# AtharvRN/dflash

Measured on AMD Instinct MI355X. Metric: accepted_tokens_per_sec, higher is better.
Workload: dtype bf16

## Files before the change

### dflash_amd/_lib.py

```python
from __future__ import annotations

import ctypes as C
import os

import torch

HERE = os.path.dirname(os.path.abspath(__file__))
LIB_PATH = os.environ.get("DFL_LIB_PATH") or os.path.join(HERE, "lib", "libdflash_hip.so")

_p, _i, _i64, _f, _u64 = C.c_void_p, C.c_int, C.c_int64, C.c_float, C.c_uint64


class Rows(C.Structure):
    _fields_ = [("frag", C.c_void_p), ("rows", C.c_void_p), ("ld", C.c_int64), ("ss", C.c_void_p),
                ("nss", C.c_int32), ("norm_w", C.c_void_p), ("eps", C.c_float), ("valid_word", C.c_int32),
                ("mode", C.c_int32)]


_r = C.POINTER(Rows)


class RowsBatch(C.Structure):
    _fields_ = [("r0", Rows), ("frag_stride", C.c_int64), ("rows_stride", C.c_int64), ("ss_stride", C.c_int64)]


_rb = C.POINTER(RowsBatch)

W_BF16, W_E4M3, W_BF16X13 = 0, 1, 2


class Weight(C.Structure):
    _fields_ = [("wp", C.c_void_p), ("scale", C.c_void_p), ("format", C.c_int32)]


_w = C.POINTER(Weight)

SIGNATURES = {
    "dfl_version": (_i, []),
    "dfl_last_error": (C.c_char_p, []),
    "dfl_pack_weight": (_i, [_p, _p, _i, _i, _p]),
    "dfl_pack_weight_gateup": (_i, [_p, _p, _p, _i, _i, _p]),
    "dfl_set_dyn": (_i, [_p, _i, _i, _i, _i, _p]),
    "dfl_set_dyn2": (_i, [_p, _i, _i, _i, _i, _p]),
# ... 114 lines not shown
```

### dflash_amd/csrc/gemm_skinny.hip

```cpp
#include "gemm_rows.h"
#include "dfl_rng.h"

namespace {

struct GemmArgs {
  const bf16x8 *wp;
  int KS;
  int ntiles;
  int nfr;
  int nch;
  int nhalf;
  int gx;
  const int32_t *dyn;
  RowSrc src[2];
  float *out;
  int ldo;
  bf16_t *act;
  const int32_t *elist, *n_active;
  int npp;
  int row0, nrows;
  int nrows_word;
  float *best_val;
  int *best_idx;
  float *best2_val;
// ... 49 lines not shown
  a.gx = (int)b.gx;
  a.nch = CHUNKED ? (int)b.nch_nss : 1;
  a.nrows_word = (int)b.nrows_word1 - 1;
  RowSrc &s = a.src[0];
  s.frag = reinterpret_cast<const bf16x8 *>(x);
  s.rows = reinterpret_cast<const bf16_t *>(x);
  s.ld = ld;
  s.ss = ss;
  s.nw = nw;
  s.mode = (int)b.mode;
  s.valid_word = (int)b.valid_word1 - 1;
  if (NORM) s.nss = (int)b.nch_nss;
  return a;
}

template <bool CHUNKED>
bool gemm_head(GemmHead &h, const GemmArgs &a) {
  const RowSrc &s = a.src[0];
  HeadBits b{};
  b.KS = a.KS;
  b.nfr = a.nfr;
  b.mode = s.mode;
  b.valid_word1 = s.valid_word < 0 ? 0 : s.valid_word + 1;
  b.nrows_word1 = a.nrows_word < 0 ? 0 : a.nrows_word + 1;
  b.gx = a.gx;
  b.nhalf = a.nhalf;
  const int nch_nss = CHUNKED ? a.nch : (s.mode == 2 ? s.nss : 0);
  b.nch_nss = nch_nss;
  const int64_t ld = s.mode == 0 ? 0 : s.ld;
  const bool fits = (int)b.KS == a.KS && (int)b.nfr == a.nfr && (int)b.mode == s.mode && (int)b.gx == a.gx &&
// ... 19 lines not shown
#ifdef DFL_GEMM_STAMPS
__device__ unsigned long long g_gstamps[8];
__device__ unsigned long long g_wgstamps[256][4];
#define GSTAMP(i)                                                                         \
  do {                                                                                    \
    if (threadIdx.x == 0 && blockIdx.x == 0 && blockIdx.y == 0) g_gstamps[i] = __builtin_amdgcn_s_memrealtime(); \
    if (threadIdx.x == 0 && blockIdx.y == 0 && blockIdx.x < 256 && ((i) == 0 || (i) == 4 || (i) == 5))            \
      g_wgstamps[blockIdx.x][(i) == 0 ? 0 : (i) - 3] = __builtin_amdgcn_s_memrealtime();                           \
  } while (0)
#else
#define GSTAMP(i)
#endif

constexpr int gemm_fr(int MT, bool CHUNKED) { return CHUNKED ? 4 : (MT == 1 ? 8 : 4); }

template <int MT, bool CHUNKED, int EPI, bool NORM, bool W8 = false, bool W13 = false>
__device__ __forceinline__ void gemm_body(const GemmArgs &a, const SampleArgs &sa) {
  GSTAMP(0);
  static_assert(!W13 || (MT == 1 && !W8), "W13: the single-tile bf16 kernels only");
  static_assert(!W13 || !CHUNKED || (EPI == EPI_RESID && !NORM), "W13, K-chunked: the residual launch only");
  constexpr int FR = gemm_fr(MT, CHUNKED);
  constexpr int NW = W13 ? (CHUNKED ? 3 : 6) : (W8 ? FR / 2 : FR);
  __shared__ float red[2][16][MT][256];
  __shared__ float ssred[NORM ? MT : 1][16][16];
  __shared__ bf16x8 nwl[NORM ? MT : 1][NORM ? 512 : 1];

  const int tid = threadIdx.x;
  const int w = __builtin_amdgcn_readfirstlane(tid >> 6);
  const int l = tid & 63;

  auto ks0_of = [&](int c) { return ((blockIdx.y * a.nch + c) * 16 + w) * a.nfr; };
  auto nf_of = [&](int c) {
    int nf = a.KS - ks0_of(c);
    return nf < 0 ? 0 : (nf > a.nfr ? a.nfr : nf);
  };

  const int stride = a.gx;
  constexpr bool SILU = EPI == EPI_SILU || EPI == EPI_SILU_E;
  constexpr bool moe = EPI == EPI_SILU_E;
  const int nwhole = (!SILU && (int)blockIdx.x < a.ntiles) ? (a.ntiles - 1 - (int)blockIdx.x) / stride + 1 : 0;
  const bool has_half = !SILU && (int)blockIdx.x < a.nhalf;
  const int myhalf = (int)blockIdx.x & 1;
  auto half_of = [&](int j) -> int { return (!SILU && j >= nwhole) ? myhalf : -1; };
  auto tile_of = [&](int j) -> int {
    if (!SILU) return j < nwhole ? (int)blockIdx.x + j * stride : a.ntiles + ((int)blockIdx.x >> 1);
    int p = (int)blockIdx.x + (j >> 1) * stride;
    if (moe) p = a.elist[p / a.npp] * a.npp + p % a.npp;
    return 2 * p + (j & 1);
  };

  bf16x8 wA[NW], wB[NW];
  float scA = 1.f, scB = 1.f;
  W13Extra exA{}, exB{};
  bf16x8 xA[MT][FR], xB[MT][FR];
  bf16x8 xr[MT][FR];

  const int nf0 = nf_of(0);
  const int ngroups = SILU ? a.ntiles >> 1 : a.ntiles;
  int nseq;
  if (SILU) {
    const int npairs = moe ? a.n_active[0] * a.npp : a.ntiles >> 1;
    nseq = (int)blockIdx.x < npairs ? 2 * ((npairs - 1 - (int)blockIdx.x) / stride + 1) : 0;
  } else {
    nseq = nwhole + (has_half ? 1 : 0);
  }
  const int nitems = nseq * a.nch;

  int nv[MT];
  auto read_nv = [&]() {
#pragma unroll
    for (int mt = 0; mt < MT; ++mt) {
      const RowSrc &s0 = a.src[mt];
      nv[mt] = (s0.valid_word >= 0 && a.dyn) ? a.dyn[s0.valid_word] : 16;
    }
  };

  float best = -INFINITY;
  int bestn = 0x7fffffff;
  float second = -INFINITY;
  float gate_sum = 0.f;
  int arg_rows = 0;
  int pos_row0 = 0, rng_extra = 0;

  auto load_item_x = [&](bf16x8(&xb)[MT][FR], int c) {
    const int ks0 = ks0_of(c);
    int ks[FR];
#pragma unroll
    for (int f = 0; f < FR; ++f) ks[f] = ks0 + f < a.KS ? ks0 + f : a.KS - 1;
    bf16x8 wv[MT][FR];
#pragma unroll
    for (int mt = 0; mt < MT; ++mt)
#pragma unroll
      for (int f = 0; f < FR; ++f) wv[mt][f] = xb[mt][f] = (bf16x8){0, 0, 0, 0, 0, 0, 0, 0};
#pragma unroll
    for (int mt = 0; mt < MT; ++mt) issue_x<FR, false>(a.src[mt], ks, l, nv[mt], xb[mt], wv[mt]);
  };
// ... 103 lines not shown
          const bool keep = ks0c + f < a.KS && (a.src[mt].mode == 0 || (l & 15) < nv[mt]);
          xv = keep ? xb[mt][f] : (bf16x8){0, 0, 0, 0, 0, 0, 0, 0};
        }
        bf16x8 wf;
        if constexpr (W13 && CHUNKED)
          wf = w13_frag(wr, ex.sg[0], ex.meta, f, l);
        else if constexpr (W13)
          wf = w13_frag(wr, ex, f, l);
        else
          wf = weight_frag<W8>(wr, f);
        acc[mt] = __builtin_amdgcn_mfma_f32_16x16x32_bf16(wf, xv, acc[mt], 0, 0, 0);
      }
    if (!CHUNKED || c == a.nch - 1) finish(t, pos, wsc);
  };

  const int first_tile = (SILU || nwhole > 0) ? (int)blockIdx.x : a.ntiles + ((int)blockIdx.x >> 1);
  const int first_half = (SILU || nwhole > 0) ? -1 : myhalf;
  const bool first_live = SILU ? (int)blockIdx.x < ngroups : (nwhole > 0 || has_half);
  auto ask_resid0 = [&]() {
    if (PREF) {
      const int ff = tid & 255;
      resid0 = a.h_io[(int64_t)(ff >> 4) * a.ldh + first_tile * 16 + (ff & 15)];
    }
  };

  read_nv();
  int arg_word = 0;
  const bool arg_dyn = (EPI == EPI_ARGMAX || EPI == EPI_SAMPLE) && a.dyn && a.nrows_word >= 0;
  if (arg_dyn) arg_word = a.dyn[a.nrows_word];
  if (EPI == EPI_SAMPLE) {
    const int base = sa.pos_dyn ? sa.pos_dyn[sa.pos_word] : sa.pos_base;
    pos_row0 = base + sa.pos_add;
    rng_extra = sa.rng_stream == (int)DFL_RNG_DRAFT ? base : 0;
// ... 87 lines not shown
        }
    }
    GSTAMP(2);
#pragma unroll
    for (int mt = 0; mt < MT; ++mt) {
      if (NORM)
        finish_xl<FR>(a.src[mt], ks, take, l, nv[mt], rstd[mt], raw[mt], nwl[mt], xr[mt]);
      else
        finish_x<FR, false>(a.src[mt], take, l, nv[mt], 1.f, raw[mt], wv0[mt], xr[mt]);
    }
  } else {
    if constexpr (W8)
      load_w8(wA, scA, first_tile, ks0_of(0), first_live ? nf0 : 0, first_half);
    else if constexpr (W13)
      load_w13(wA, exA, first_tile, ks0_of(0), first_live ? nf0 : 0, first_half, 0);
    else if (nitems > 0 || !moe)
      load_ksteps<FR>(wA, a.wp + ((size_t)first_tile * a.KS + ks0_of(0)) * 64, first_live ? nf0 : 0, l, first_half);
    GSTAMP(6);
    load_item_x(xA, 0);
    ask_resid0();
    GSTAMP(1);
    GSTAMP(2);
  }

  if (EPI == EPI_ARGMAX || EPI == EPI_SAMPLE) arg_rows = arg_dyn ? arg_word - a.row0 : a.nrows;
  GSTAMP(3);
  if (nitems > 0) {
    int j = 0, c = 0;
    for (int i = 0;; i += 2) {
      int jn = j, cn = c + 1;
      if (cn == a.nch) {
        cn = 0;
        ++jn;
      }
      if (i + 1 < nitems) load_item(wB, scB, exB, xB, tile_of(jn), cn, half_of(jn));
      process(wA, scA, exA, xA, tile_of(j), c, j);
      if (i == 0) GSTAMP(4);
      if (i + 1 >= nitems) break;
      int j2 = jn, c2 = cn + 1;
// ... 40 lines not shown
template <bool CHUNKED, int EPI, bool NORM>
__global__ __launch_bounds__(1024) void k_gemm_w8(GEMM_HEAD_PARAMS, GemmArgs rest) {
  gemm_body<1, CHUNKED, EPI, NORM, true>(with_head<CHUNKED, NORM>(rest, GEMM_HEAD_NAMES), SampleArgs{});
}

template <int EPI, bool NORM>
__global__ __launch_bounds__(1024) void k_gemm_w13(GEMM_HEAD_PARAMS, GemmArgs rest) {
  gemm_body<1, false, EPI, NORM, false, true>(with_head<false, NORM>(rest, GEMM_HEAD_NAMES), SampleArgs{});
}

template <int EPI>
__global__ __launch_bounds__(1024) void k_gemm_w13c(GEMM_HEAD_PARAMS, GemmArgs rest) {
  gemm_body<1, true, EPI, false, false, true>(with_head<true, false>(rest, GEMM_HEAD_NAMES), SampleArgs{});
}

template <bool NORM>
__global__ __launch_bounds__(1024) void k_gemm_s(GEMM_HEAD_PARAMS, GemmArgs rest, SampleArgs sa) {
  gemm_body<1, false, EPI_SAMPLE, NORM>(with_head<false, NORM>(rest, GEMM_HEAD_NAMES), sa);
}

template <bool NORM>
__global__ __launch_bounds__(1024) void k_gemm_s_w8(GEMM_HEAD_PARAMS, GemmArgs rest, SampleArgs sa) {
  gemm_body<1, false, EPI_SAMPLE, NORM, true>(with_head<false, NORM>(rest, GEMM_HEAD_NAMES), sa);
}

template <int MT, bool CHUNKED, int EPI, bool W8 = false>
bool launch_gemm(GemmArgs &a, dim3 grid, hipStream_t stream) {
  bool norm = false;
  for (int mt = 0; mt < MT; ++mt) norm |= a.src[mt].mode == 2;
  a.gx = (int)grid.x;
  GemmHead h;
  if (!gemm_head<CHUNKED>(h, a)) return false;
  if constexpr (W8) {
    static_assert(MT == 1, "the W8 kernels take one 16-row tile");
    if (!a.wscale || a.KS % 2 || a.nfr % 2) {
      dfl_set_error("skinny GEMM (fp8): needs a scale vector, K %% 64 == 0 and an even share per wave (K=%d, nfr=%d)",
                    a.KS * 32, a.nfr);
      return false;
    }
    if constexpr (!CHUNKED) {
      if (norm) {
        hipLaunchKernelGGL((k_gemm_w8<false, EPI, true>), grid, dim3(1024), 0, stream, GEMM_HEAD_OF(h), a);
        return true;
      }
    }
    hipLaunchKernelGGL((k_gemm_w8<CHUNKED, EPI, false>), grid, dim3(1024), 0, stream, GEMM_HEAD_OF(h), a);
    return true;
  }
  if constexpr (!CHUNKED) {
    if (norm) {
      hipLaunchKernelGGL((k_gemm<MT, false, EPI, true>), grid, dim3(1024), 0, stream, GEMM_HEAD_OF(h), a);
      return true;
    }
  }
  hipLaunchKernelGGL((k_gemm<MT, CHUNKED, EPI, false>), grid, dim3(1024), 0, stream, GEMM_HEAD_OF(h), a);
  return true;
}

static int64_t w13_quads_bytes(int N, int K) { return (int64_t)(N / 16) * (K / 128) * W13_QUAD_BYTES; }

template <int EPI>
bool launch_gemm_w13(const char *who, GemmArgs &a, const dfl_weight *w, int N, dim3 grid, hipStream_t stream) {
  if (w->scale) {
    dfl_set_error("%s: a DFL_W_BF16X13 weight takes no scale vector (the bases and patch words follow the codes)", who);
    return false;
  }
  if (a.KS % 64 || a.nfr % 4 || a.nfr * 16 != a.KS) {
    dfl_set_error("%s: DFL_W_BF16X13 covers K = 2048 and K = 4096 only (whole quads of four k-steps per wave; K=%d, %d k-steps "
                  "per wave)", who, a.KS * 32, a.nfr);
    return false;
  }
  a.wscale = reinterpret_cast<const float *>(reinterpret_cast<const char *>(w->wp) + w13_quads_bytes(N, a.KS * 32));
  a.gx = (int)grid.x;
  GemmHead h;
  if (!gemm_head<false>(h, a)) return false;
  if (a.src[0].mode == 2)
    hipLaunchKernelGGL((k_gemm_w13<EPI, true>), grid, dim3(1024), 0, stream, GEMM_HEAD_OF(h), a);
  else
    hipLaunchKernelGGL((k_gemm_w13<EPI, false>), grid, dim3(1024), 0, stream, GEMM_HEAD_OF(h), a);
  return true;
}

__global__ __launch_bounds__(64) void k_argmax_finish(const float *best_val, const int *best_idx, const float *best2_val,
                                                      int nblk, int row0, int nrows, const int32_t *dyn, int nrows_word,
                                                      int64_t *out_ids, int out_off, float *margin_out) {
  int rows = nrows;
  if (dyn && nrows_word >= 0) rows = dyn[nrows_word] - row0;
  const int m = row0 + blockIdx.x;
  if ((int)blockIdx.x >= rows) return;
  float bv = -INFINITY, sv = -INFINITY;
// ... 179 lines not shown
  a.out = out;
  a.ldo = N;
  int gx1 = 0;
  if (ksplit == 1) plan_tiles(a, N / 16, true, gx1);
  dim3 grid(ksplit == 1 ? gx1 : grid_x_for(a.ntiles, ksplit), ksplit);
  const bool ok = mt == 1 ? launch_gemm<1, false, EPI_F32>(a, grid, (hipStream_t)stream)
                          : launch_gemm<2, false, EPI_F32>(a, grid, (hipStream_t)stream);
  if (!ok) return DFL_EINVAL;
  DFL_CHECK_LAUNCH("dfl_gemm_f32");
  return DFL_OK;
}

namespace {
template <bool W8, bool W13 = false>
int gemm_silu_mul_impl(const char *who, const dfl_weight *w, const dfl_rows *x, int I, int K, void *act_frag,
                       const int32_t *dyn, void *stream) {
  DFL_REQUIRE(w->wp && act_frag && (!W8 || w->scale), "%s: null pointer", who);
  DFL_REQUIRE(I > 0 && K > 0 && I % 16 == 0 && K % (W8 ? 64 : 32) == 0, "%s: need I%%16==0, K%%%d==0", who, W8 ? 64 : 32);
  const int KS = K / 32;
  DFL_REQUIRE(KS <= 16 * 8, "%s: K=%d needs a K split, which the fused activation cannot take", who, K);
  GemmArgs a{};
  if (!fill_src(a.src[0], x, K, who)) return DFL_EINVAL;
  a.wp = (const bf16x8 *)w->wp;
  a.wscale = w->scale;
  a.dyn = dyn;
  a.KS = KS;
  a.ntiles = 2 * (I / 16);
  a.nfr = (KS + 15) / 16;
  if (W8) a.nfr += a.nfr & 1;
  a.nch = 1;
  a.act = (bf16_t *)act_frag;
  if constexpr (W13) {
    if (!launch_gemm_w13<EPI_SILU>(who, a, w, 2 * I, dim3(grid_x_for(I / 16), 1), (hipStream_t)stream)) return DFL_EINVAL;
  } else if (!launch_gemm<1, false, EPI_SILU, W8>(a, dim3(grid_x_for(I / 16), 1), (hipStream_t)stream)) {
    return DFL_EINVAL;
  }
  DFL_CHECK_LAUNCH(who);
  return DFL_OK;
}
}

extern "C" int dfl_gemm_silu_mul(const dfl_weight *w_gateup, const dfl_rows *x, int I, int K, void *act_frag,
                                 const int32_t *dyn, void *stream) {
  const char *who = "dfl_gemm_silu_mul";
  if (w_gateup && w_gateup->format == DFL_W_BF16X13)
    return gemm_silu_mul_impl<false, true>(who, w_gateup, x, I, K, act_frag, dyn, stream);
  if (!weight_ok(who, w_gateup)) return DFL_EINVAL;
  return w_gateup->format == DFL_W_BF16 ? gemm_silu_mul_impl<false>(who, w_gateup, x, I, K, act_frag, dyn, stream)
                                        : gemm_silu_mul_impl<true>(who, w_gateup, x, I, K, act_frag, dyn, stream);
}

extern "C" int dfl_gemm_silu_mul_experts(const void *wp_gateup, int64_t wp_expert_stride, const dfl_rows *x, int E, int I, int K,
                                         void *act_frag, int64_t act_expert_stride, const int32_t *list,
                                         const int32_t *n_active, const int32_t *dyn, void *stream) {
  DFL_REQUIRE(wp_gateup && act_frag && list && n_active, "dfl_gemm_silu_mul_experts: null pointer");
  DFL_REQUIRE(E >= 1 && E <= 1024 && I > 0 && K > 0 && I % 16 == 0 && K % 32 == 0, "dfl_gemm_silu_mul_experts: bad shape");
  DFL_REQUIRE(wp_expert_stride == (int64_t)2 * I * K && act_expert_stride == (int64_t)16 * I,
              "dfl_gemm_silu_mul_experts: the experts' weights and outputs must lie back to back (strides %lld, %lld)",
              (long long)wp_expert_stride, (long long)act_expert_stride);
  const int KS = K / 32;
  DFL_REQUIRE(KS <= 16 * 8, "dfl_gemm_silu_mul_experts: K=%d exceeds 4096", K);
  GemmArgs a{};
  if (!fill_src(a.src[0], x, K, "dfl_gemm_silu_mul_experts")) return DFL_EINVAL;
  a.wp = (const bf16x8 *)wp_gateup;
// ... 4 lines not shown
  a.nch = 1;
  a.act = (bf16_t *)act_frag;
  a.elist = list;
  a.n_active = n_active;
  a.npp = I / 16;
  if (!launch_gemm<1, false, EPI_SILU_E>(a, dim3(256, 1), (hipStream_t)stream)) return DFL_EINVAL;
  DFL_CHECK_LAUNCH("dfl_gemm_silu_mul_experts");
  return DFL_OK;
}

extern "C" int64_t dfl_argmax_ws_bytes(void) { return 256 * 16 * (int64_t)(2 * sizeof(float) + sizeof(int)); }

namespace {
int gemm_argmax_impl(const char *who, const dfl_weight *w, const dfl_rows *x, int V, int K, int row0, int nrows,
                     const int32_t *dyn, int nrows_dyn_word, void *ws, int64_t *out_ids, int out_off, void *logits,
                     float *margin_out, hipEvent_t ev0, hipEvent_t ev1, void *stream, const SampleArgs *smp = nullptr) {
  const bool w8 = w->format == DFL_W_E4M3, w13 = w->format == DFL_W_BF16X13;
  DFL_REQUIRE(w->wp && ws && out_ids && (!w8 || w->scale), "%s: null pointer", who);
  DFL_REQUIRE(V > 0 && K > 0 && V % 16 == 0 && K % (w8 ? 64 : 32) == 0, "%s: need V%%16==0, K%%%d==0 (V=%d K=%d)", who,
              w8 ? 64 : 32, V, K);
  DFL_REQUIRE(row0 >= 0 && nrows >= 0 && row0 + nrows <= 16, "%s: rows [%d,%d) outside the 16-row tile", who, row0,
              row0 + nrows);
  const int KS = K / 32;
  DFL_REQUIRE(KS <= 16 * 8, "%s: K=%d exceeds 4096 (argmax needs finished sums)", who, K);
  GemmArgs a{};
  if (!fill_src(a.src[0], x, K, who)) return DFL_EINVAL;
  a.wp = (const bf16x8 *)w->wp;
  a.dyn = dyn;
  a.KS = KS;
  a.ntiles = V / 16;
  a.nfr = (KS + 15) / 16;
// ... 13 lines not shown
  if (ev0) (void)hipEventRecord(ev0, (hipStream_t)stream);
  if (smp) {
    a.gx = gx;
    GemmHead h;
    if (!gemm_head<false>(h, a)) return DFL_EINVAL;
    if (w8) {
      if (a.src[0].mode == 2)
        hipLaunchKernelGGL(k_gemm_s_w8<true>, dim3(gx, 1), dim3(1024), 0, (hipStream_t)stream, GEMM_HEAD_OF(h), a, *smp);
      else
        hipLaunchKernelGGL(k_gemm_s_w8<false>, dim3(gx, 1), dim3(1024), 0, (hipStream_t)stream, GEMM_HEAD_OF(h), a, *smp);
    } else if (a.src[0].mode == 2)
      hipLaunchKernelGGL(k_gemm_s<true>, dim3(gx, 1), dim3(1024), 0, (hipStream_t)stream, GEMM_HEAD_OF(h), a, *smp);
    else
      hipLaunchKernelGGL(k_gemm_s<false>, dim3(gx, 1), dim3(1024), 0, (hipStream_t)stream, GEMM_HEAD_OF(h), a, *smp);
  } else if (w13) {
    if (!launch_gemm_w13<EPI_ARGMAX>(who, a, w, V, dim3(gx, 1), (hipStream_t)stream)) return DFL_EINVAL;
  } else if (w8) {
    if (!launch_gemm<1, false, EPI_ARGMAX, true>(a, dim3(gx, 1), (hipStream_t)stream)) return DFL_EINVAL;
  } else {
    if (!launch_gemm<1, false, EPI_ARGMAX>(a, dim3(gx, 1), (hipStream_t)stream)) return DFL_EINVAL;
  }
  if (ev1) (void)hipEventRecord(ev1, (hipStream_t)stream);
  hipLaunchKernelGGL(k_argmax_finish, dim3(16), dim3(64), 0, (hipStream_t)stream, a.best_val, a.best_idx, a.best2_val, gx,
                     row0, nrows, dyn, nrows_dyn_word, out_ids, out_off, margin_out);
  DFL_CHECK_LAUNCH(who);
  return DFL_OK;
}
}

extern "C" int dfl_gemm_argmax(const dfl_weight *w, const dfl_rows *x, int V, int K, int row0, int nrows,
                               const int32_t *dyn, int nrows_dyn_word, void *ws, int64_t *out_ids, int out_off,
                               void *logits, float *margin_out, void *ev_start, void *ev_end, void *stream) {
  const char *who = "dfl_gemm_argmax";
  if (!(w && w->format == DFL_W_BF16X13) && !weight_ok(who, w)) return DFL_EINVAL;
  return gemm_argmax_impl(who, w, x, V, K, row0, nrows, dyn, nrows_dyn_word, ws, out_ids, out_off, logits, margin_out,
                          (hipEvent_t)ev_start, (hipEvent_t)ev_end, stream);
}

extern "C" int dfl_gemm_sample(const dfl_weight *w, const dfl_rows *x, int V, int K, int row0, int nrows,
                               const int32_t *dyn, int nrows_dyn_word, void *ws, int64_t *out_ids, int out_off,
                               void *logits, float *margin_out, uint64_t seed, float inv_t, int rng_stream,
                               const int32_t *pos_dyn, int pos_word, int pos_base, int pos_add, void *stream) {
  const char *who = "dfl_gemm_sample";
  if (!weight_ok(who, w)) return DFL_EINVAL;
  DFL_REQUIRE(w->wp && (w->format == DFL_W_BF16 || w->scale) && ws && out_ids, "%s: null pointer", who);
  DFL_REQUIRE(inv_t > 0.f && inv_t <= 1e5f, "%s: inv_t=%g outside (0, 1e5]", who, (double)inv_t);
  DFL_REQUIRE(rng_stream == (int)DFL_RNG_TARGET || rng_stream == (int)DFL_RNG_DRAFT, "%s: unknown stream %d", who,
              rng_stream);
  DFL_REQUIRE(!pos_dyn || (pos_word >= 0 && pos_word < DFL_DYN_WORDS), "%s: pos_word=%d outside the record", who, pos_word);
  const SampleArgs smp{seed, inv_t, rng_stream, pos_dyn, pos_word, pos_base, pos_add};
  return gemm_argmax_impl(who, w, x, V, K, row0, nrows, dyn, nrows_dyn_word, ws, out_ids, out_off, logits, margin_out,
                          nullptr, nullptr, stream, &smp);
}


namespace {
template <bool W8, bool W13 = false>
int gemm_resid_impl(const char *who, const dfl_weight *w, const dfl_rows *x, int N, int K, void *h_io, int64_t ldh,
                    int add_residual, void *tap, int64_t ldtap, float *ss_out, const int32_t *dyn, void *stream) {
  DFL_REQUIRE(w->wp && h_io && (!W8 || w->scale), "%s: null pointer", who);
  DFL_REQUIRE(N > 0 && K > 0 && N % 16 == 0 && K % (W8 ? 64 : 32) == 0, "%s: need N%%16==0, K%%%d==0 (N=%d K=%d)", who,
              W8 ? 64 : 32, N, K);
  DFL_REQUIRE(ldh >= N && (!tap || ldtap >= N), "%s: row strides shorter than N", who);
  const int KS = K / 32;
  GemmArgs a{};
  if (!fill_src(a.src[0], x, K, who)) return DFL_EINVAL;
  a.wp = (const bf16x8 *)w->wp;
  a.wscale = w->scale;
  a.dyn = dyn;
  a.KS = KS;
  a.ntiles = N / 16;
  a.h_io = (bf16_t *)h_io;
  a.ldh = ldh;
  a.add_resid = add_residual ? 1 : 0;
  a.tap = (bf16_t *)tap;
  a.ldtap = ldtap;
  a.ss_out = ss_out;
  int gx = 0;
  plan_tiles(a, N / 16, KS <= 16 * 8 && !ss_out, gx);
  const dim3 grid(gx, 1);
  if (KS <= 16 * 8) {
    a.nfr = (KS + 15) / 16;
    if (W8) a.nfr += a.nfr & 1;
    a.nch = 1;
    if (!launch_gemm<1, false, EPI_RESID, W8>(a, grid, (hipStream_t)stream)) return DFL_EINVAL;
  } else {
    DFL_REQUIRE(a.src[0].mode != 2, "%s: a normalised source needs K <= 4096", who);
    a.nfr = 4;
    a.nch = (KS + 63) / 64;
    if constexpr (W13) {
      a.wscale = reinterpret_cast<const float *>(reinterpret_cast<const char *>(w->wp) + w13_quads_bytes(N, K));
      a.gx = (int)grid.x;
      GemmHead h;
      if (!gemm_head<true>(h, a)) return DFL_EINVAL;
      hipLaunchKernelGGL((k_gemm_w13c<EPI_RESID>), grid, dim3(1024), 0, (hipStream_t)stream, GEMM_HEAD_OF(h), a);
    } else if (!launch_gemm<1, true, EPI_RESID, W8>(a, grid, (hipStream_t)stream)) {
      return DFL_EINVAL;
    }
  }
  DFL_CHECK_LAUNCH(who);
  return DFL_OK;
}
}

extern "C" int dfl_gemm_resid(const dfl_weight *w, const dfl_rows *x, int N, int K, void *h_io, int64_t ldh,
                              int add_residual, void *tap, int64_t ldtap, float *ss_out, const int32_t *dyn,
                              void *stream) {
  const char *who = "dfl_gemm_resid";
  if (w && w->format == DFL_W_BF16X13 && K > 4096 && K % 2048 == 0) {
    DFL_REQUIRE(!w->scale, "%s: a DFL_W_BF16X13 weight takes no scale vector (the bases and patch words follow the codes)", who);
    return gemm_resid_impl<false, true>(who, w, x, N, K, h_io, ldh, add_residual, tap, ldtap, ss_out, dyn, stream);
  }
  if (!weight_ok(who, w)) return DFL_EINVAL;
  return w->format == DFL_W_BF16
             ? gemm_resid_impl<false>(who, w, x, N, K, h_io, ldh, add_residual, tap, ldtap, ss_out, dyn, stream)
             : gemm_resid_impl<true>(who, w, x, N, K, h_io, ldh, add_residual, tap, ldtap, ss_out, dyn, stream);
}
```

### dflash_amd/ops.py

```python
from __future__ import annotations

from types import SimpleNamespace
from typing import NamedTuple, Optional

import torch

from ._lib import W_BF16, W_BF16X13, W_E4M3, Rows, Weight, check, lib

BF16, F32, I32, I64 = torch.bfloat16, torch.float32, torch.int32, torch.int64
DYN_S, DYN_TAU, DYN_BS, DYN_POS0, DYN_START, DYN_STOP, DYN_CYCLE = range(7)


def _stream() -> int:
    return torch.cuda.current_stream().cuda_stream


def _p(t: Optional[torch.Tensor], dtype=None, name="tensor") -> Optional[int]:
    if t is None:
        return None
    if not t.is_cuda:
        raise RuntimeError(f"dflash_amd: {name} must be a GPU tensor (got {t.device}); there is no CPU path")
    if dtype is not None and t.dtype != dtype:
        raise TypeError(f"dflash_amd: {name} must be {dtype}, got {t.dtype}")
    if not t.is_contiguous():
# ... 225 lines not shown
    return hit[3]


def bf16x13_report() -> dict:
    live = [v for v in _x13_twins.values() if v[0]() is not None]
    return {"packed": sum(v[3] is not None for v in live), "kept_bf16": sum(v[3] is None for v in live),
            "patched_items": sum(v[4]["patched"] for v in live), "refused_items": sum(v[4]["refused"] for v in live)}


def check_stream_format(stream_format: str) -> bool:
    if stream_format not in STREAM_FORMATS:
        raise ValueError(f"stream_format must be one of {STREAM_FORMATS}, got {stream_format!r}")
    return stream_format == "auto"


def _w(wp, N: int, K: int, name: str) -> Weight:
    if isinstance(wp, Bf16x13Weight):
        if (wp.N, wp.K) != (N, K):
            raise ValueError(f"dflash_amd: {name} is a bf16x13 weight of {wp.N} x {wp.K}, the launch asks for {N} x {K}")
        return Weight(_p(wp.data, U8, name), None, W_BF16X13)
    if not isinstance(wp, Fp8Weight):
        return Weight(_p(wp, BF16, name), None, W_BF16)
    if (wp.N, wp.K) != (N, K):
        raise ValueError(f"dflash_amd: {name} is an fp8 weight of {wp.N} x {wp.K}, the launch asks for {N} x {K}")
    return Weight(_p(wp.wp, U8, name), _p(wp.scale, F32, name + ".scale"), W_E4M3)


def _we(wp, E: int, N: int, K: int, name: str):
    if not isinstance(wp, Fp8Experts):
        assert wp.dim() == 2 and wp.is_contiguous()
        return Weight(_p(wp, BF16, name), None, W_BF16), wp
    if (wp.E, wp.N, wp.K) != (E, N, K):
        raise ValueError(f"dflash_amd: {name} holds fp8 experts of {wp.E} x {wp.N} x {wp.K}, the launch asks for "
                         f"{E} x {N} x {K}")
    return Weight(_p(wp.wp, U8, name), _p(wp.scale, F32, name + ".scale"), W_E4M3), wp.wp


def set_dyn(dyn: torch.Tensor, S: int, tau: int, bs: int, pos0: int) -> None:
    check(lib().dfl_set_dyn(_p(dyn, I32, "dyn"), S, tau, bs, pos0, _stream()), "dfl_set_dyn")

# ... 73 lines not shown
    ntiles, ks_steps = N // 16, K // 32
    best, best_score = None, None
    for ks in range(min_ksplit(K, mt), 17):
        nfr = -(-ks_steps // (16 * ks))
        if nfr < 2 and ks > min_ksplit(K, mt):
            break
        gx_max = max(1, 256 // ks)
        per_wg = -(-ntiles // gx_max)
        fill = (ntiles * ks) / (256.0 * per_wg)
        score = (round(min(fill, 1.0), 3), min(per_wg, 2), -ks)
        if best_score is None or score > best_score:
            best, best_score = ks, score
    return best


def gemm_silu_mul(wp_gu, x, I: int, K: int, act_frag: torch.Tensor, dyn=None) -> None:
    assert act_frag.numel() >= 16 * I
    check(lib().dfl_gemm_silu_mul(_w(wp_gu, 2 * I, K, "wp_gu"), _src(x).ref, I, K, _p(act_frag, BF16, "act"),
                                  _p(dyn, I32, "dyn"), _stream()), "dfl_gemm_silu_mul")


def argmax_ws(device) -> torch.Tensor:
    return torch.empty(lib().dfl_argmax_ws_bytes(), dtype=torch.uint8, device=device)


def gemm_argmax(wp, x, V: int, K: int, row0: int, nrows: int, ws, out_ids: torch.Tensor, out_off: int = 0,
                dyn=None, nrows_dyn_word: int = -1, logits: Optional[torch.Tensor] = None,
                margins: Optional[torch.Tensor] = None, events=None) -> None:
    if logits is not None:
        assert logits.numel() >= 16 * V
    if margins is not None:
        assert margins.numel() >= out_off + nrows
    ev_start, ev_end = (None, None) if events is None else (events[0].cuda_event, events[1].cuda_event)
    check(lib().dfl_gemm_argmax(_w(wp, V, K, "wp"), _src(x).ref, V, K, row0, nrows, _p(dyn, I32, "dyn"), nrows_dyn_word,
                                _p(ws), _p(out_ids, I64, "out_ids"), out_off, _p(logits, BF16, "logits"),
                                _p(margins, F32, "margins"), ev_start, ev_end, _stream()), "dfl_gemm_argmax")


RNG_TARGET, RNG_DRAFT = 0, 1


def _seed64(seed: int) -> int:
    return int(seed) & 0xFFFFFFFFFFFFFFFF


def inv_temperature(temperature: float) -> float:
    import numpy as np
    return float(np.float32(1.0 / float(temperature)))

# ... 355 lines not shown
    if out_ids is not None:
        assert out_ids.stride(-1) == 1 and out_ids.shape[-1] >= out_off + n_out, "out_ids"
        assert out_ids.dim() == 2 and out_ids.shape[0] >= tiles or out_ids.dim() == 1 and tiles == 1, "out_ids"
        out_stride = out_ids.stride(0) if out_ids.dim() == 2 else 0
    if dyn is not None:
        assert dyn.numel() >= 8 * tiles
    check(lib().dfl_logit_bias_rows(logits.data_ptr(), out.data_ptr(), ld, tile_stride, tiles, V, row0, nrows,
                                    _p(dyn, I32, "dyn"), nrows_dyn_word, tiles_per_req, bias.data_ptr(), bias.stride(0),
                                    mp_p, mp_v, _p(stop_ids, I64, "stop_ids") if n_stop else None, n_stop, pos_word,
                                    pos_base, pos_add, _p(out_ids, I64, "out_ids"), out_stride, out_off, _stream()),
          "dfl_logit_bias_rows")
    return out


def gemm_resid(wp, x, N: int, K: int, h_io: torch.Tensor, *, add_residual: bool, ss_out=None, tap=None,
               dyn=None) -> None:
    assert h_io.is_cuda and h_io.dtype == BF16 and h_io.stride(1) == 1
    tp, ldt = None, 0
    if tap is not None:
        assert tap.is_cuda and tap.dtype == BF16 and tap.stride(1) == 1
        tp, ldt = tap.data_ptr(), tap.stride(0)
    if ss_out is not None:
        assert ss_out.numel() >= N
    check(lib().dfl_gemm_resid(_w(wp, N, K, "wp"), _src(x).ref, N, K, h_io.data_ptr(), h_io.stride(0),
                               int(add_residual), tp, ldt, _p(ss_out, F32, "ss_out"), _p(dyn, I32, "dyn"), _stream()),
          "dfl_gemm_resid")


def embed_rows(embed, ids, h_out, H: int, ss_out, dyn=None, dyn_word: int = 0) -> None:
    check(lib().dfl_embed_rows(_p(embed, BF16, "embed"), _p(ids, I64, "ids"), _p(h_out, BF16, "h_out"), H,
                               _p(ss_out, F32, "ss_out"), _p(dyn, I32, "dyn"), dyn_word, _stream()), "dfl_embed_rows")


def norm_pack(*, norm_w, frag, H: int, eps: float, part=None, nsplit=0, part_split=0, ldp=0, row_off=0,
              resid_in=None, embed=None, ids=None, h_out=None, h_out2=None, ld2=0, dyn=None, dyn_word=0) -> None:
    p2 = None
    if h_out2 is not None:
        assert h_out2.is_cuda and h_out2.dtype == BF16 and h_out2.stride(-1) == 1
        p2 = h_out2.data_ptr()
# ... 597 lines not shown
```

### include/dflash_hip.h

```cpp
#ifndef DFLASH_HIP_H
#define DFLASH_HIP_H

#include <stdint.h>

#ifdef __cplusplus
extern "C" {
#endif

#define DFL_ABI_VERSION 1

#define DFL_OK 0
#define DFL_EINVAL (-22)
#define DFL_ELAUNCH (-5)

#define DFL_DYN_WORDS 8
#define DFL_DYN_S 0
#define DFL_DYN_TAU 1
#define DFL_DYN_BS 2
#define DFL_DYN_POS0 3
#define DFL_DYN_START 4
#define DFL_DYN_STOP 5
#define DFL_DYN_CYCLE 6

typedef struct dfl_rows {
  const void *frag;
  const void *rows;
  int64_t ld;
  const float *ss;
  int32_t nss;
  const void *norm_w;
  float eps;
  int32_t valid_word;
  int32_t mode;
} dfl_rows;

enum { DFL_W_BF16 = 0, DFL_W_E4M3 = 1, DFL_W_BF16X13 = 2 };
typedef struct dfl_weight {
  const void *wp;
  const float *scale;
  int32_t format;
} dfl_weight;

int dfl_version(void);
const char *dfl_last_error(void);


int dfl_pack_weight(const void *w, void *wp, int N, int K, void *stream);
int dfl_pack_weight_gateup(const void *gate, const void *up, void *wp, int I, int K, void *stream);
int dfl_pack_weight_fp8(const void *q, void *wp8, int N, int K, void *stream);
int dfl_pack_weight_gateup_fp8(const void *gate_q, const void *up_q, void *wp8, int I, int K, void *stream);

// ... 250 lines not shown
```

Baseline: 1831.

## Add shape-specialised skinny GEMM kernels with compile-time K and deferred counters

Adds templated 'form' variants of the skinny GEMM kernel for the residual (bf16) and SiLU (bf16x13) launches in which K steps, fragments per wave, chunk count, source mode, row stride and optionally grid width are compile-time constants when K is 64 or 128 steps. In these variants the item counting and argmax/finish state initialisation move after the first weight and activation loads are issued, which shortens the launch prologue and lowers register pressure. The aim is to cut per-launch integer overhead and let the compiler fold address arithmetic in latency-bound decode GEMMs. A GENERIC weight-format flag lets callers force the old path, at the cost of more kernel instantiations.

```diff
diff --git a/dflash_amd/_lib.py b/dflash_amd/_lib.py
--- a/dflash_amd/_lib.py
+++ b/dflash_amd/_lib.py
@@ -27,6 +27,7 @@
 _rb = C.POINTER(RowsBatch)
 
 W_BF16, W_E4M3, W_BF16X13 = 0, 1, 2
+W_GENERIC = 0x100
 
 
 class Weight(C.Structure):
diff --git a/dflash_amd/csrc/gemm_skinny.hip b/dflash_amd/csrc/gemm_skinny.hip
--- a/dflash_amd/csrc/gemm_skinny.hip
+++ b/dflash_amd/csrc/gemm_skinny.hip
@@ -87,6 +87,28 @@
   return a;
 }
 
+struct NoShape {
+  static constexpr bool shaped = false;
+};
+template <int KS_, int NFR_, int NCH_, int MODE_, bool G256_>
+struct Shape {
+  static constexpr bool shaped = true, g256 = G256_;
+  static constexpr int KS = KS_, nfr = NFR_, nch = NCH_, mode = MODE_;
+};
+
+template <class SH>
+__device__ __forceinline__ GemmArgs with_shape(GemmArgs a) {
+  if constexpr (SH::shaped) {
+    a.KS = SH::KS;
+    a.nfr = SH::nfr;
+    a.nch = SH::nch;
+    a.src[0].mode = SH::mode;
+    if (SH::mode != 0) a.src[0].ld = SH::KS * 32;
+    if (SH::g256) a.gx = 256;
+  }
+  return a;
+}
+
 template <bool CHUNKED>
 bool gemm_head(GemmHead &h, const GemmArgs &a) {
   const RowSrc &s = a.src[0];
@@ -136,9 +158,12 @@
 
 constexpr int gemm_fr(int MT, bool CHUNKED) { return CHUNKED ? 4 : (MT == 1 ? 8 : 4); }
 
-template <int MT, bool CHUNKED, int EPI, bool NORM, bool W8 = false, bool W13 = false>
+template <int MT, bool CHUNKED, int EPI, bool NORM, bool W8 = false, bool W13 = false, class SH = NoShape>
 __device__ __forceinline__ void gemm_body(const GemmArgs &a, const SampleArgs &sa) {
   GSTAMP(0);
+  static_assert(!SH::shaped || (MT == 1 && !W8 && !CHUNKED && EPI != EPI_F32 && EPI != EPI_SILU_E), "shape forms: one tile, one K pass, bf16 / W13, grid.y == 1");
+  constexpr bool LATE = SH::shaped;
+  const unsigned by = SH::shaped ? 0u : blockIdx.y;
   static_assert(!W13 || (MT == 1 && !W8), "W13: the single-tile bf16 kernels only");
   static_assert(!W13 || !CHUNKED || (EPI == EPI_RESID && !NORM), "W13, K-chunked: the residual launch only");
   constexpr int FR = gemm_fr(MT, CHUNKED);
@@ -151,8 +176,9 @@
   const int w = __builtin_amdgcn_readfirstlane(tid >> 6);
   const int l = tid & 63;
 
-  auto ks0_of = [&](int c) { return ((blockIdx.y * a.nch + c) * 16 + w) * a.nfr; };
+  auto ks0_of = [&](int c) { return ((by * a.nch + c) * 16 + w) * a.nfr; };
   auto nf_of = [&](int c) {
+    if constexpr (SH::shaped) return (int)SH::nfr;
     int nf = a.KS - ks0_of(c);
     return nf < 0 ? 0 : (nf > a.nfr ? a.nfr : nf);
   };
@@ -160,7 +186,9 @@
   const int stride = a.gx;
   constexpr bool SILU = EPI == EPI_SILU || EPI == EPI_SILU_E;
   constexpr bool moe = EPI == EPI_SILU_E;
-  const int nwhole = (!SILU && (int)blockIdx.x < a.ntiles) ? (a.ntiles - 1 - (int)blockIdx.x) / stride + 1 : 0;
+  int nwhole;
+  auto count_whole = [&]() { nwhole = (!SILU && (int)blockIdx.x < a.ntiles) ? (a.ntiles - 1 - (int)blockIdx.x) / stride + 1 : 0; };
+  if (!LATE) count_whole();
   const bool has_half = !SILU && (int)blockIdx.x < a.nhalf;
   const int myhalf = (int)blockIdx.x & 1;
   auto half_of = [&](int j) -> int { return (!SILU && j >= nwhole) ? myhalf : -1; };
@@ -179,14 +207,17 @@
 
   const int nf0 = nf_of(0);
   const int ngroups = SILU ? a.ntiles >> 1 : a.ntiles;
-  int nseq;
-  if (SILU) {
-    const int npairs = moe ? a.n_active[0] * a.npp : a.ntiles >> 1;
-    nseq = (int)blockIdx.x < npairs ? 2 * ((npairs - 1 - (int)blockIdx.x) / stride + 1) : 0;
-  } else {
-    nseq = nwhole + (has_half ? 1 : 0);
-  }
-  const int nitems = nseq * a.nch;
+  int nseq, nitems;
+  auto count_items = [&]() {
+    if (SILU) {
+      const int npairs = moe ? a.n_active[0] * a.npp : a.ntiles >> 1;
+      nseq = (int)blockIdx.x < npairs ? 2 * ((npairs - 1 - (int)blockIdx.x) / stride + 1) : 0;
+    } else {
+      nseq = nwhole + (has_half ? 1 : 0);
+    }
+    nitems = nseq * a.nch;
+  };
+  if (!LATE) count_items();
 
   int nv[MT];
   auto read_nv = [&]() {
@@ -197,11 +228,18 @@
     }
   };
 
-  float best = -INFINITY;
-  int bestn = 0x7fffffff;
-  float second = -INFINITY;
-  float gate_sum = 0.f;
-  int arg_rows = 0;
+  float best, second;
+  int bestn;
+  float gate_sum;
+  int arg_rows;
+  auto init_finish = [&]() {
+    best = -INFINITY;
+    bestn = 0x7fffffff;
+    second = -INFINITY;
+    gate_sum = 0.f;
+    arg_rows = 0;
+  };
+  if (!LATE) init_finish();
   int pos_row0 = 0, rng_extra = 0;
 
   auto load_item_x = [&](bf16x8(&xb)[MT][FR], int c) {
@@ -335,9 +373,10 @@
     if (!CHUNKED || c == a.nch - 1) finish(t, pos, wsc);
   };
 
-  const int first_tile = (SILU || nwhole > 0) ? (int)blockIdx.x : a.ntiles + ((int)blockIdx.x >> 1);
-  const int first_half = (SILU || nwhole > 0) ? -1 : myhalf;
-  const bool first_live = SILU ? (int)blockIdx.x < ngroups : (nwhole > 0 || has_half);
+  const bool has_whole = LATE ? (!SILU && (int)blockIdx.x < a.ntiles) : nwhole > 0;
+  const int first_tile = (SILU || has_whole) ? (int)blockIdx.x : a.ntiles + ((int)blockIdx.x >> 1);
+  const int first_half = (SILU || has_whole) ? -1 : myhalf;
+  const bool first_live = SILU ? (int)blockIdx.x < ngroups : (has_whole || has_half);
   auto ask_resid0 = [&]() {
     if (PREF) {
       const int ff = tid & 255;
@@ -455,7 +494,7 @@
       load_w8(wA, scA, first_tile, ks0_of(0), first_live ? nf0 : 0, first_half);
     else if constexpr (W13)
       load_w13(wA, exA, first_tile, ks0_of(0), first_live ? nf0 : 0, first_half, 0);
-    else if (nitems > 0 || !moe)
+    else if (!moe || nitems > 0)
       load_ksteps<FR>(wA, a.wp + ((size_t)first_tile * a.KS + ks0_of(0)) * 64, first_live ? nf0 : 0, l, first_half);
     GSTAMP(6);
     load_item_x(xA, 0);
@@ -464,6 +503,11 @@
     GSTAMP(2);
   }
 
+  if (LATE) {
+    count_whole();
+    count_items();
+    init_finish();
+  }
   if (EPI == EPI_ARGMAX || EPI == EPI_SAMPLE) arg_rows = arg_dyn ? arg_word - a.row0 : a.nrows;
   GSTAMP(3);
   if (nitems > 0) {
@@ -534,6 +578,11 @@
   gemm_body<1, true, EPI, false, false, true>(with_head<true, false>(rest, GEMM_HEAD_NAMES), SampleArgs{});
 }
 
+template <int EPI, bool NORM, bool W13, class SH>
+__global__ __launch_bounds__(1024) void k_gemm_form(GEMM_HEAD_PARAMS, GemmArgs rest) {
+  gemm_body<1, false, EPI, NORM, false, W13, SH>(with_shape<SH>(with_head<false, NORM>(rest, GEMM_HEAD_NAMES)), SampleArgs{});
+}
+
 template <bool NORM>
 __global__ __launch_bounds__(1024) void k_gemm_s(GEMM_HEAD_PARAMS, GemmArgs rest, SampleArgs sa) {
   gemm_body<1, false, EPI_SAMPLE, NORM>(with_head<false, NORM>(rest, GEMM_HEAD_NAMES), sa);
@@ -544,13 +593,55 @@
   gemm_body<1, false, EPI_SAMPLE, NORM, true>(with_head<false, NORM>(rest, GEMM_HEAD_NAMES), sa);
 }
 
+template <int EPI, bool W13, int MODE, int KS, bool G256>
+void launch_form_as(const GemmArgs &a, const GemmHead &h, dim3 grid, hipStream_t stream) {
+  using SH = Shape<KS, KS / 16, 1, MODE, G256>;
+  hipLaunchKernelGGL((k_gemm_form<EPI, MODE == 2, W13, SH>), grid, dim3(1024), 0, stream, GEMM_HEAD_OF(h), a);
+}
+template <int EPI, bool W13, int MODE>
+bool launch_form(const GemmArgs &a, const GemmHead &h, dim3 grid, hipStream_t stream) {
+  constexpr int KS0 = 64;
+  const RowSrc &s = a.src[0];
+  if (grid.y != 1 || s.mode != MODE || (MODE != 0 && s.ld != (int64_t)a.KS * 32)) return false;
+  if (a.nch != 1 || a.KS != 16 * a.nfr) return false;
+  if (a.KS != KS0 && a.KS != 2 * KS0) return false;
+  const bool g256 = grid.x == 256;
+  if (a.KS == KS0)
+    g256 ? launch_form_as<EPI, W13, MODE, KS0, true>(a, h, grid, stream)
+         : launch_form_as<EPI, W13, MODE, KS0, false>(a, h, grid, stream);
+  else
+    g256 ? launch_form_as<EPI, W13, MODE, 2 * KS0, true>(a, h, grid, stream)
+         : launch_form_as<EPI, W13, MODE, 2 * KS0, false>(a, h, grid, stream);
+  return true;
+}
+template <bool CHUNKED, int EPI, bool W13>
+bool launch_any_form(const GemmArgs &a, const GemmHead &h, dim3 grid, hipStream_t stream) {
+  if constexpr (!CHUNKED && EPI == EPI_RESID && !W13)
+    return launch_form<EPI_RESID, false, 0>(a, h, grid, stream);
+  else if constexpr (!CHUNKED && EPI == EPI_SILU && W13)
+    return launch_form<EPI_SILU, true, 2>(a, h, grid, stream);
+  else
+    return false;
+}
+
+static bool take_generic_flag(const dfl_weight *&w, dfl_weight &local) {
+  if (!w || !(w->format & DFL_W_GENERIC)) return false;
+  local = *w;
+  local.format &= ~(int32_t)DFL_W_GENERIC;
+  w = &local;
+  return true;
+}
+
 template <int MT, bool CHUNKED, int EPI, bool W8 = false>
-bool launch_gemm(GemmArgs &a, dim3 grid, hipStream_t stream) {
+bool launch_gemm(GemmArgs &a, dim3 grid, hipStream_t stream, bool generic = false) {
   bool norm = false;
   for (int mt = 0; mt < MT; ++mt) norm |= a.src[mt].mode == 2;
   a.gx = (int)grid.x;
   GemmHead h;
   if (!gemm_head<CHUNKED>(h, a)) return false;
+  if constexpr (MT == 1 && !W8 && (EPI == EPI_RESID || EPI == EPI_SILU || EPI == EPI_ARGMAX)) {
+    if (!generic && launch_any_form<CHUNKED, EPI, false>(a, h, grid, stream)) return true;
+  }
   if constexpr (W8) {
     static_assert(MT == 1, "the W8 kernels take one 16-row tile");
     if (!a.wscale || a.KS % 2 || a.nfr % 2) {
@@ -580,7 +671,7 @@
 static int64_t w13_quads_bytes(int N, int K) { return (int64_t)(N / 16) * (K / 128) * W13_QUAD_BYTES; }
 
 template <int EPI>
-bool launch_gemm_w13(const char *who, GemmArgs &a, const dfl_weight *w, int N, dim3 grid, hipStream_t stream) {
+bool launch_gemm_w13(const char *who, GemmArgs &a, const dfl_weight *w, int N, dim3 grid, hipStream_t stream, bool generic) {
   if (w->scale) {
     dfl_set_error("%s: a DFL_W_BF16X13 weight takes no scale vector (the bases and patch words follow the codes)", who);
     return false;
@@ -594,6 +685,7 @@
   a.gx = (int)grid.x;
   GemmHead h;
   if (!gemm_head<false>(h, a)) return false;
+  if (!generic && launch_any_form<false, EPI, true>(a, h, grid, stream)) return true;
   if (a.src[0].mode == 2)
     hipLaunchKernelGGL((k_gemm_w13<EPI, true>), grid, dim3(1024), 0, stream, GEMM_HEAD_OF(h), a);
   else
@@ -803,7 +895,7 @@
 namespace {
 template <bool W8, bool W13 = false>
 int gemm_silu_mul_impl(const char *who, const dfl_weight *w, const dfl_rows *x, int I, int K, void *act_frag,
-                       const int32_t *dyn, void *stream) {
+                       const int32_t *dyn, void *stream, bool generic) {
   DFL_REQUIRE(w->wp && act_frag && (!W8 || w->scale), "%s: null pointer", who);
   DFL_REQUIRE(I > 0 && K > 0 && I % 16 == 0 && K % (W8 ? 64 : 32) == 0, "%s: need I%%16==0, K%%%d==0", who, W8 ? 64 : 32);
   const int KS = K / 32;
@@ -820,8 +912,8 @@
   a.nch = 1;
   a.act = (bf16_t *)act_frag;
   if constexpr (W13) {
-    if (!launch_gemm_w13<EPI_SILU>(who, a, w, 2 * I, dim3(grid_x_for(I / 16), 1), (hipStream_t)stream)) return DFL_EINVAL;
-  } else if (!launch_gemm<1, false, EPI_SILU, W8>(a, dim3(grid_x_for(I / 16), 1), (hipStream_t)stream)) {
+    if (!launch_gemm_w13<EPI_SILU>(who, a, w, 2 * I, dim3(grid_x_for(I / 16), 1), (hipStream_t)stream, generic)) return DFL_EINVAL;
+  } else if (!launch_gemm<1, false, EPI_SILU, W8>(a, dim3(grid_x_for(I / 16), 1), (hipStream_t)stream, generic)) {
     return DFL_EINVAL;
   }
   DFL_CHECK_LAUNCH(who);
@@ -832,11 +924,13 @@
 extern "C" int dfl_gemm_silu_mul(const dfl_weight *w_gateup, const dfl_rows *x, int I, int K, void *act_frag,
                                  const int32_t *dyn, void *stream) {
   const char *who = "dfl_gemm_silu_mul";
+  dfl_weight wl;
+  const bool generic = take_generic_flag(w_gateup, wl);
   if (w_gateup && w_gateup->format == DFL_W_BF16X13)
-    return gemm_silu_mul_impl<false, true>(who, w_gateup, x, I, K, act_frag, dyn, stream);
+    return gemm_silu_mul_impl<false, true>(who, w_gateup, x, I, K, act_frag, dyn, stream, generic);
   if (!weight_ok(who, w_gateup)) return DFL_EINVAL;
-  return w_gateup->format == DFL_W_BF16 ? gemm_silu_mul_impl<false>(who, w_gateup, x, I, K, act_frag, dyn, stream)
-                                        : gemm_silu_mul_impl<true>(who, w_gateup, x, I, K, act_frag, dyn, stream);
+  return w_gateup->format == DFL_W_BF16 ? gemm_silu_mul_impl<false>(who, w_gateup, x, I, K, act_frag, dyn, stream, generic)
+                                        : gemm_silu_mul_impl<true>(who, w_gateup, x, I, K, act_frag, dyn, stream, generic);
 }
 
 extern "C" int dfl_gemm_silu_mul_experts(const void *wp_gateup, int64_t wp_expert_stride, const dfl_rows *x, int E, int I, int K,
@@ -871,7 +965,8 @@
 namespace {
 int gemm_argmax_impl(const char *who, const dfl_weight *w, const dfl_rows *x, int V, int K, int row0, int nrows,
                      const int32_t *dyn, int nrows_dyn_word, void *ws, int64_t *out_ids, int out_off, void *logits,
-                     float *margin_out, hipEvent_t ev0, hipEvent_t ev1, void *stream, const SampleArgs *smp = nullptr) {
+                     float *margin_out, hipEvent_t ev0, hipEvent_t ev1, void *stream, const SampleArgs *smp = nullptr,
+                     bool generic = false) {
   const bool w8 = w->format == DFL_W_E4M3, w13 = w->format == DFL_W_BF16X13;
   DFL_REQUIRE(w->wp && ws && out_ids && (!w8 || w->scale), "%s: null pointer", who);
   DFL_REQUIRE(V > 0 && K > 0 && V % 16 == 0 && K % (w8 ? 64 : 32) == 0, "%s: need V%%16==0, K%%%d==0 (V=%d K=%d)", who,
@@ -915,11 +1010,11 @@
     else
       hipLaunchKernelGGL(k_gemm_s<false>, dim3(gx, 1), dim3(1024), 0, (hipStream_t)stream, GEMM_HEAD_OF(h), a, *smp);
   } else if (w13) {
-    if (!launch_gemm_w13<EPI_ARGMAX>(who, a, w, V, dim3(gx, 1), (hipStream_t)stream)) return DFL_EINVAL;
+    if (!launch_gemm_w13<EPI_ARGMAX>(who, a, w, V, dim3(gx, 1), (hipStream_t)stream, generic)) return DFL_EINVAL;
   } else if (w8) {
     if (!launch_gemm<1, false, EPI_ARGMAX, true>(a, dim3(gx, 1), (hipStream_t)stream)) return DFL_EINVAL;
   } else {
-    if (!launch_gemm<1, false, EPI_ARGMAX>(a, dim3(gx, 1), (hipStream_t)stream)) return DFL_EINVAL;
+    if (!launch_gemm<1, false, EPI_ARGMAX>(a, dim3(gx, 1), (hipStream_t)stream, generic)) return DFL_EINVAL;
   }
   if (ev1) (void)hipEventRecord(ev1, (hipStream_t)stream);
   hipLaunchKernelGGL(k_argmax_finish, dim3(16), dim3(64), 0, (hipStream_t)stream, a.best_val, a.best_idx, a.best2_val, gx,
@@ -933,9 +1028,11 @@
                                const int32_t *dyn, int nrows_dyn_word, void *ws, int64_t *out_ids, int out_off,
                                void *logits, float *margin_out, void *ev_start, void *ev_end, void *stream) {
   const char *who = "dfl_gemm_argmax";
+  dfl_weight wl;
+  const bool generic = take_generic_flag(w, wl);
   if (!(w && w->format == DFL_W_BF16X13) && !weight_ok(who, w)) return DFL_EINVAL;
   return gemm_argmax_impl(who, w, x, V, K, row0, nrows, dyn, nrows_dyn_word, ws, out_ids, out_off, logits, margin_out,
-                          (hipEvent_t)ev_start, (hipEvent_t)ev_end, stream);
+                          (hipEvent_t)ev_start, (hipEvent_t)ev_end, stream, nullptr, generic);
 }
 
 extern "C" int dfl_gemm_sample(const dfl_weight *w, const dfl_rows *x, int V, int K, int row0, int nrows,
@@ -958,7 +1055,7 @@
 namespace {
 template <bool W8, bool W13 = false>
 int gemm_resid_impl(const char *who, const dfl_weight *w, const dfl_rows *x, int N, int K, void *h_io, int64_t ldh,
-                    int add_residual, void *tap, int64_t ldtap, float *ss_out, const int32_t *dyn, void *stream) {
+                    int add_residual, void *tap, int64_t ldtap, float *ss_out, const int32_t *dyn, void *stream, bool generic) {
   DFL_REQUIRE(w->wp && h_io && (!W8 || w->scale), "%s: null pointer", who);
   DFL_REQUIRE(N > 0 && K > 0 && N % 16 == 0 && K % (W8 ? 64 : 32) == 0, "%s: need N%%16==0, K%%%d==0 (N=%d K=%d)", who,
               W8 ? 64 : 32, N, K);
@@ -984,7 +1081,7 @@
     a.nfr = (KS + 15) / 16;
     if (W8) a.nfr += a.nfr & 1;
     a.nch = 1;
-    if (!launch_gemm<1, false, EPI_RESID, W8>(a, grid, (hipStream_t)stream)) return DFL_EINVAL;
+    if (!launch_gemm<1, false, EPI_RESID, W8>(a, grid, (hipStream_t)stream, generic)) return DFL_EINVAL;
   } else {
     DFL_REQUIRE(a.src[0].mode != 2, "%s: a normalised source needs K <= 4096", who);
     a.nfr = 4;
@@ -995,7 +1092,7 @@
       GemmHead h;
       if (!gemm_head<true>(h, a)) return DFL_EINVAL;
       hipLaunchKernelGGL((k_gemm_w13c<EPI_RESID>), grid, dim3(1024), 0, (hipStream_t)stream, GEMM_HEAD_OF(h), a);
-    } else if (!launch_gemm<1, true, EPI_RESID, W8>(a, grid, (hipStream_t)stream)) {
+    } else if (!launch_gemm<1, true, EPI_RESID, W8>(a, grid, (hipStream_t)stream, generic)) {
       return DFL_EINVAL;
     }
   }
@@ -1008,12 +1105,14 @@
                               int add_residual, void *tap, int64_t ldtap, float *ss_out, const int32_t *dyn,
                               void *stream) {
   const char *who = "dfl_gemm_resid";
+  dfl_weight wl;
+  const bool generic = take_generic_flag(w, wl);
   if (w && w->format == DFL_W_BF16X13 && K > 4096 && K % 2048 == 0) {
     DFL_REQUIRE(!w->scale, "%s: a DFL_W_BF16X13 weight takes no scale vector (the bases and patch words follow the codes)", who);
-    return gemm_resid_impl<false, true>(who, w, x, N, K, h_io, ldh, add_residual, tap, ldtap, ss_out, dyn, stream);
+    return gemm_resid_impl<false, true>(who, w, x, N, K, h_io, ldh, add_residual, tap, ldtap, ss_out, dyn, stream, generic);
   }
   if (!weight_ok(who, w)) return DFL_EINVAL;
   return w->format == DFL_W_BF16
-             ? gemm_resid_impl<false>(who, w, x, N, K, h_io, ldh, add_residual, tap, ldtap, ss_out, dyn, stream)
-             : gemm_resid_impl<true>(who, w, x, N, K, h_io, ldh, add_residual, tap, ldtap, ss_out, dyn, stream);
-}
+             ? gemm_resid_impl<false>(who, w, x, N, K, h_io, ldh, add_residual, tap, ldtap, ss_out, dyn, stream, generic)
+             : gemm_resid_impl<true>(who, w, x, N, K, h_io, ldh, add_residual, tap, ldtap, ss_out, dyn, stream, generic);
+}
diff --git a/dflash_amd/ops.py b/dflash_amd/ops.py
--- a/dflash_amd/ops.py
+++ b/dflash_amd/ops.py
@@ -5,7 +5,7 @@
 
 import torch
 
-from ._lib import W_BF16, W_BF16X13, W_E4M3, Rows, Weight, check, lib
+from ._lib import W_BF16, W_BF16X13, W_E4M3, W_GENERIC, Rows, Weight, check, lib
 
 BF16, F32, I32, I64 = torch.bfloat16, torch.float32, torch.int32, torch.int64
 DYN_S, DYN_TAU, DYN_BS, DYN_POS0, DYN_START, DYN_STOP, DYN_CYCLE = range(7)
@@ -263,16 +263,17 @@
     return stream_format == "auto"
 
 
-def _w(wp, N: int, K: int, name: str) -> Weight:
+def _w(wp, N: int, K: int, name: str, generic: bool = False) -> Weight:
+    flag = W_GENERIC if generic else 0
     if isinstance(wp, Bf16x13Weight):
         if (wp.N, wp.K) != (N, K):
             raise ValueError(f"dflash_amd: {name} is a bf16x13 weight of {wp.N} x {wp.K}, the launch asks for {N} x {K}")
-        return Weight(_p(wp.data, U8, name), None, W_BF16X13)
+        return Weight(_p(wp.data, U8, name), None, W_BF16X13 | flag)
     if not isinstance(wp, Fp8Weight):
-        return Weight(_p(wp, BF16, name), None, W_BF16)
+        return Weight(_p(wp, BF16, name), None, W_BF16 | flag)
     if (wp.N, wp.K) != (N, K):
         raise ValueError(f"dflash_amd: {name} is an fp8 weight of {wp.N} x {wp.K}, the launch asks for {N} x {K}")
-    return Weight(_p(wp.wp, U8, name), _p(wp.scale, F32, name + ".scale"), W_E4M3)
+    return Weight(_p(wp.wp, U8, name), _p(wp.scale, F32, name + ".scale"), W_E4M3 | flag)
 
 
 def _we(wp, E: int, N: int, K: int, name: str):
@@ -376,9 +377,9 @@
     return best
 
 
-def gemm_silu_mul(wp_gu, x, I: int, K: int, act_frag: torch.Tensor, dyn=None) -> None:
+def gemm_silu_mul(wp_gu, x, I: int, K: int, act_frag: torch.Tensor, dyn=None, *, generic: bool = False) -> None:
     assert act_frag.numel() >= 16 * I
-    check(lib().dfl_gemm_silu_mul(_w(wp_gu, 2 * I, K, "wp_gu"), _src(x).ref, I, K, _p(act_frag, BF16, "act"),
+    check(lib().dfl_gemm_silu_mul(_w(wp_gu, 2 * I, K, "wp_gu", generic), _src(x).ref, I, K, _p(act_frag, BF16, "act"),
                                   _p(dyn, I32, "dyn"), _stream()), "dfl_gemm_silu_mul")
 
 
@@ -388,13 +389,13 @@
 
 def gemm_argmax(wp, x, V: int, K: int, row0: int, nrows: int, ws, out_ids: torch.Tensor, out_off: int = 0,
                 dyn=None, nrows_dyn_word: int = -1, logits: Optional[torch.Tensor] = None,
-                margins: Optional[torch.Tensor] = None, events=None) -> None:
+                margins: Optional[torch.Tensor] = None, events=None, *, generic: bool = False) -> None:
     if logits is not None:
         assert logits.numel() >= 16 * V
     if margins is not None:
         assert margins.numel() >= out_off + nrows
     ev_start, ev_end = (None, None) if events is None else (events[0].cuda_event, events[1].cuda_event)
-    check(lib().dfl_gemm_argmax(_w(wp, V, K, "wp"), _src(x).ref, V, K, row0, nrows, _p(dyn, I32, "dyn"), nrows_dyn_word,
+    check(lib().dfl_gemm_argmax(_w(wp, V, K, "wp", generic), _src(x).ref, V, K, row0, nrows, _p(dyn, I32, "dyn"), nrows_dyn_word,
                                 _p(ws), _p(out_ids, I64, "out_ids"), out_off, _p(logits, BF16, "logits"),
                                 _p(margins, F32, "margins"), ev_start, ev_end, _stream()), "dfl_gemm_argmax")
 
@@ -780,7 +781,7 @@
 
 
 def gemm_resid(wp, x, N: int, K: int, h_io: torch.Tensor, *, add_residual: bool, ss_out=None, tap=None,
-               dyn=None) -> None:
+               dyn=None, generic: bool = False) -> None:
     assert h_io.is_cuda and h_io.dtype == BF16 and h_io.stride(1) == 1
     tp, ldt = None, 0
     if tap is not None:
@@ -788,7 +789,7 @@
         tp, ldt = tap.data_ptr(), tap.stride(0)
     if ss_out is not None:
         assert ss_out.numel() >= N
-    check(lib().dfl_gemm_resid(_w(wp, N, K, "wp"), _src(x).ref, N, K, h_io.data_ptr(), h_io.stride(0),
+    check(lib().dfl_gemm_resid(_w(wp, N, K, "wp", generic), _src(x).ref, N, K, h_io.data_ptr(), h_io.stride(0),
                                int(add_residual), tp, ldt, _p(ss_out, F32, "ss_out"), _p(dyn, I32, "dyn"), _stream()),
           "dfl_gemm_resid")
 
diff --git a/include/dflash_hip.h b/include/dflash_hip.h
--- a/include/dflash_hip.h
+++ b/include/dflash_hip.h
@@ -35,6 +35,7 @@
 } dfl_rows;
 
 enum { DFL_W_BF16 = 0, DFL_W_E4M3 = 1, DFL_W_BF16X13 = 2 };
+enum { DFL_W_GENERIC = 0x100 };
 typedef struct dfl_weight {
   const void *wp;
   const float *scale;
```

Measured after the change: 1828. Within noise of the previous version (-0.1%).
